# VanshJP/ShippingEnv

Measured on AMD Instinct MI355X. Metric: env-steps/sec at N=2^20 parallel envs per GPU (config 3: full step, 5 default ports; K steps in the steady state after a 1000-step pre-roll; config3_literal: the survey's 1000 steps from reset), higher is better.
Workload: dtype f64+int (fuel f64; reward computed in f64, stored f32 after one rounding; positions/cargo int)

## Files before the change

### shippingenv_amd/csrc/shipenv.hip

```cpp
#include <hip/hip_runtime.h>

#include <math.h>
#include <stdint.h>
#include <stdio.h>
#include <stdlib.h>
#include <string.h>

#include <algorithm>
#include <atomic>
#include <initializer_list>
#include <string>
#include <vector>

#include "../../include/shipenv.h"
#include "navfield.h"
#include "philox.h"
#include "step_lean.h"

#ifndef SHIPENV_TRACE
#define SHIPENV_TRACE 0
#endif

using namespace shipenv;

namespace {

constexpr int kBlock = 256;
constexpr int kStepBlock = 256;
constexpr int kEnvsPerThread = 4;
constexpr int kMaxBlocks = 2048;
constexpr int kStepBlocks = 32768;

constexpr uint32_t kUsedFuelGate = SE_USED_FUEL_GATE, kUsedLossType = SE_USED_LOSS_TYPE,
                   kUsedBeta = SE_USED_BETA, kUsedArrive = SE_USED_ARRIVE, kUsedMoved = SE_USED_MOVED;

constexpr double kFuelInit = 200.0;
constexpr double kMaxCargo = 50.0;

#include "world.h"
#include "env_core.h"
#include "step_io.h"
#include "step_group.h"
#include "step_agent.h"
#include "step_kernel.h"
#include "step_seq.h"
#include "views.h"
#include "rollout.h"
#include "episode.h"
#include "plan.h"
}

struct se_env {
    int device = 0;
    int64_t n = 0, env_base = 0;
    WorldDims dims{};
    uint64_t seed = 0;
    uint32_t flags = 0;
    uint64_t step_t = 0, epoch = 0;
    std::vector<uint8_t> water;
    std::vector<int32_t> port_x, port_y;
    uint32_t* d_world = nullptr;
    int64_t seg = 0;
    int64_t iters = 1;
    size_t world_cap = 0;
    uint64_t world_version = 0;
    int32_t cmax = 0, fmax = 0;
    int32_t stock_cargo_max = 0;
    se_state st{};
    bool bound = false;
    double* d_slab = nullptr;
    int32_t* d_offsets = nullptr;
    int grid = 0;
    int64_t nseg = 0;
    int64_t nslab = 0;
    uint8_t* d_mask_tmpl = nullptr;
    size_t mask_tmpl_cap = 0;
    uint64_t mask_tmpl_version = 0;
    int mask_ntmpl = 0;
    bool mask_tiled = false;
    int32_t done_pad = 1;
    bool nt_loads = false;
    bool seq_fuse = true;
    int32_t seq_max_steps = 1024;
    bool seq_gate_pool = true;
    bool seq_ring = true;
};

struct se_host {
    WorldDims dims{};
    std::vector<uint8_t> water;
    std::vector<uint32_t> img;
};

namespace {

#include "host.h"


int step_block_cap() {
    const char* v = getenv("SHIPENV_STEP_BLOCKS");
    const int c = v ? atoi(v) : 0;
    return c > 0 ? c : kStepBlocks;
}

int32_t done_pad_records(const se_env* env) {
    const char* v = getenv("SHIPENV_DONE_PAD");
    if (v) return atoi(v) == 0 ? 1 : 8;
    return env->n > (int64_t)1 << 23 ? 8 : 1;
}

bool step_nt_loads(const se_env* env) {
    const char* v = getenv("SHIPENV_NT_LOADS");
    if (v) return atoi(v) != 0;
    if (env->flags & SE_FLAG_AUTO_RESET) return env->n > (int64_t)1 << 21;
    return env->n <= (int64_t)1 << 23;
}

constexpr int32_t kSeqMaxSteps = 1024;
int32_t seq_max_steps() {
    const char* v = getenv("SHIPENV_SEQ_MAX_STEPS");
    const int c = v ? atoi(v) : 0;
    return c > 0 ? c : kSeqMaxSteps;
}
bool seq_fuse() {
    const char* v = getenv("SHIPENV_SEQ_FUSE");
    return !v || atoi(v) != 0;
}

bool seq_gate_pool() {
    const char* v = getenv("SHIPENV_SEQ_GATE_POOL");
    return !v || atoi(v) != 0;
}

bool seq_ring() {
    const char* v = getenv("SHIPENV_SEQ_RING");
    return !v || atoi(v) != 0;
}

bool mask_tiled() {
    const char* v = getenv("SHIPENV_MASK_TILED");
    return v && atoi(v) != 0;
}

int build_world_image(int H, int W, const std::vector<uint8_t>& water, int32_t P, const int32_t* px,
                      const int32_t* py, const int32_t* pf, const int32_t* pc, WorldDims& dims,
                      std::vector<uint32_t>& img) {
    if (P < 0 || P > SE_MAX_PORTS) return fail(SE_EINVAL, "P must be in [0, 254]");
    for (int i = 0; i < P; ++i) {
        if (px[i] < 0 || px[i] >= H || py[i] < 0 || py[i] >= W)
            return fail(SE_EINVAL, "Coordinates not within map");
        if (pf[i] < 0 || pc[i] < 0) return fail(SE_EINVAL, "port stocks must be >= 0");
    }
    const int cw = (H * W + 15) / 16 * 4;
    WorldDims d{H, W, P, cw};
    img.assign((size_t)d.padded(), 0u);
    uint8_t* cell = reinterpret_cast<uint8_t*>(img.data());
    for (int c = 0; c < H * W; ++c) cell[c] = water[c] ? 0 : (uint8_t)kCellGround;
    for (int i = P - 1; i >= 0; --i)
        cell[(size_t)px[i] * W + py[i]] = (uint8_t)(i + 1);
    for (int i = 0; i < P; ++i) {
        img[d.pos() + i] = (uint32_t)px[i] | ((uint32_t)py[i] << 16);
        img[d.stk() + 2 * i] = (uint32_t)pf[i];
        img[d.stk() + 2 * i + 1] = (uint32_t)pc[i];
    }
    for (int c = 0; c < 50; ++c) {
        const double q = (double)c / kMaxCargo;
        memcpy(&img[d.frac() + 2 * c], &q, sizeof q);
        img[d.gate() + c] = (uint32_t)floor(ldexp(q, 32));
    }
    img[d.gate() + 50] = 0xffffffffu;
    const int mdx[4] = {0, -1, 0, 1}, mdy[4] = {-1, 0, 1, 0};
    for (int k = 0; k < 4; ++k)
        img[d.moves() + k] = ((uint32_t)mdx[k] & 0xffffu) | (((uint32_t)mdy[k] & 0xffffu) << 16);
    double rtab[10];
    for (int k = 0; k < 8; ++k) {
        double r = 0.0;
        if (k & 4) r += -10.0;
        if (k & 2) {
            r += -5.0;
        } else {
            r += -0.0001;
            r += -1.0;
        }
        r += (k & 1) ? 2.0 : -2.0;
        rtab[k] = r;
    }
    rtab[8] = 0.05;
    rtab[9] = 0.0;
    memcpy(&img[d.rtab()], rtab, sizeof rtab);
    dims = d;
    return SE_OK;
}

int upload_world(se_env* env, int32_t P, const int32_t* px, const int32_t* py, const int32_t* pf,
                 const int32_t* pc) {
    WorldDims d{};
    std::vector<uint32_t> img;
    int rc = build_world_image(env->dims.H, env->dims.W, env->water, P, px, py, pf, pc, d, img);
    if (rc) return rc;
    std::vector<uint8_t> ring(ring_table_bytes(d.H, d.W));
    ring_table_build(d.H, d.W, reinterpret_cast<const uint8_t*>(img.data()), ring.data());
    rc = device_reserve(env->d_world, env->world_cap, (size_t)d.padded() * 4 + ring.size());
    if (rc) return rc;
    HIP_TRY(hipMemcpy(env->d_world, img.data(), (size_t)d.padded() * 4, hipMemcpyHostToDevice));
    HIP_TRY(hipMemcpy(env->d_world + d.padded(), ring.data(), ring.size(), hipMemcpyHostToDevice));
    env->dims = d;
    env->port_x.assign(px, px + P);
    env->port_y.assign(py, py + P);
    env->cmax = env->fmax = env->stock_cargo_max = 0;
    for (int i = 0; i < P; ++i) {
        env->cmax = std::max(env->cmax, std::min(pc[i], 49));
        env->fmax = std::max(env->fmax, std::min(pf[i], 199));
        env->stock_cargo_max = std::max(env->stock_cargo_max, pc[i]);
    }
    env->world_version += 1;
    env->mask_ntmpl = 1 + P;
    for (int p = 0; p < P; ++p)
        for (int q = 0; q < P; ++q) env->mask_ntmpl += (px[p] == px[q] && py[p] == py[q]) ? 1 : 0;
    return SE_OK;
}

typedef void (*StepFn)(StepArgs);
struct StepRow {
    uint32_t key;
    StepFn fn;
};
constexpr uint32_t step_key(bool typed, bool replay, bool autoreset, bool nt = false, bool rec = false, bool seq = false) {
    return typed | replay << 1 | autoreset << 2 | nt << 3 | rec << 4 | seq << 5;
}
template <bool... kFlags>
constexpr StepRow step_row() {
    return {step_key(kFlags...), step_kernel<kFlags...>};
}
template <bool... kFlags>
constexpr StepRow tail_row() {
    return {step_key(kFlags...), step_tail_kernel<kFlags...>};
}
constexpr StepRow kStepKernels[] = {
    step_row<false, false, false>(), step_row<false, false, false, true>(),
    step_row<false, false, true>(), step_row<false, false, true, true>(),
    step_row<false, false, false, false, false, true>(),
    step_row<false, false, false, true, false, true>(),
    step_row<false, false, true, false, true>(), step_row<false, false, true, true, true>(),
    step_row<false, true, false>(), step_row<true, true, false>(),
    step_row<true, false, false>(), step_row<true, false, true>(),
};
constexpr StepRow kStepTailKernels[] = {
    tail_row<false, false, false>(), tail_row<false, false, true>(), tail_row<false, true, false>(),
    tail_row<true, true, false>(),   tail_row<true, false, false>(), tail_row<true, false, true>(),
};

template <size_t kRows>
StepFn find_kernel(const StepRow (&rows)[kRows], uint32_t key) {
    for (const StepRow& r : rows)
        if (r.key == key) return r.fn;
    return nullptr;
}

StepArgs step_args(const se_env* env, const int32_t* act) {
    StepArgs A{};
    A.world = env->d_world;
    A.dims = env->dims;
    A.n = env->n;
    A.env_base = env->env_base;
    A.seed = env->seed;
    A.t = (uint32_t)env->step_t;
    A.st = env->st;
    A.act = act;
    A.iters = env->iters;
    return A;
}

int launch_step(se_env* env, bool typed, bool replay, const int32_t* act, const int32_t* a,
                const int32_t* b, se_tape* tape, void* stream, const StepRecord* rec = nullptr,
                bool seq = false) {
    int rc = check_ready(env);
    if (rc) return rc;
    if (env->n > 0 && (!act || (typed && (!a || !b)) || (replay && !tape)))
        return fail(SE_EINVAL, "null action/tape pointer");
    if (!aligned16(act) || (typed && (!aligned16(a) || !aligned16(b))))
        return fail(SE_EINVAL, "action buffers must be 16-byte aligned");
    const bool autoreset = (env->flags & SE_FLAG_AUTO_RESET) && !replay;
    if (autoreset && env->dims.P < 2) return fail(SE_EINVAL, "auto-reset needs at least two ports");
    DeviceGuard g(env->device);
    StepArgs A = step_args(env, act);
    A.act_a = a;
    A.act_b = b;
    A.tape = tape;
    if (autoreset) {
        const size_t par = (size_t)(env->step_t & 1u);
        A.done_recs = env->st.done_recs + par * (size_t)env->nseg * (size_t)env->seg;
        A.done_count = env->st.done_count + par * (size_t)env->nseg;
    }
    A.seg = env->seg;
    A.done_pad = env->done_pad;
    A.slab = env->d_slab;
    if (rec) A.rec = *rec;
    const bool agent = !typed && !replay;
    const StepFn full = find_kernel(kStepKernels, step_key(typed, replay, autoreset, agent && env->nt_loads,
                                                           rec != nullptr, agent && !autoreset && seq));
    const StepFn tail = find_kernel(kStepTailKernels, step_key(typed, replay, autoreset));
    if (!full || !tail) return fail(SE_EINVAL, "no step kernel for this kind of step");
    const hipStream_t s = (hipStream_t)stream;
    if (env->n >= kEnvsPerThread) {
        full<<<env->grid, kStepBlock, lds_bytes(env), s>>>(A);
        HIP_TRY(hipGetLastError());
    }
    if (env->n & 3) {
        tail<<<1, 64, 0, s>>>(A);
        HIP_TRY(hipGetLastError());
    }
    if (!replay) env->step_t += 1;
    return SE_OK;
}

int launch_step_seq(se_env* env, const int32_t* act, int64_t ld, int32_t steps, void* stream) {
    if (!act) return fail(SE_EINVAL, "null action/tape pointer");
    if (!aligned16(act)) return fail(SE_EINVAL, "action buffers must be 16-byte aligned");
    DeviceGuard g(env->device);
    const StepArgs A = step_args(env, act);
    const hipStream_t s = (hipStream_t)stream;
    if (env->n >= kEnvsPerThread) {
        const size_t base = lds_bytes(env) + kStockByCodeBytes;
        const bool pool = env->seq_gate_pool && base + kGatePoolBytes <= kLdsDefault;
        const size_t without = base + (pool ? kGatePoolBytes : 0);
        const uint32_t ring = env->seq_ring && ring_table_fits(env->dims.H, env->dims.W, env->dims.P, without)
                                  ? ring_table_bytes(env->dims.H, env->dims.W) : 0u;
        const size_t lds = without + ring;
        const auto kernel = pool ? (env->nt_loads ? step_seq_kernel<true, true> : step_seq_kernel<false, true>)
                                 : (env->nt_loads ? step_seq_kernel<true, false> : step_seq_kernel<false, false>);
        kernel<<<env->grid, kStepBlock, lds, s>>>(A, steps, ld, ring);
        HIP_TRY(hipGetLastError());
    }
    if (env->n & 3) {
        step_tail_seq_kernel<<<1, 64, 0, s>>>(A, steps, ld);
        HIP_TRY(hipGetLastError());
    }
    env->step_t += (uint64_t)steps;
    return SE_OK;
}

int launch_reset(se_env* env, const uint8_t* mask, const int32_t* origin, const int32_t* dest, void* stream) {
    if (env->n == 0) return SE_OK;
    DeviceGuard g(env->device);
    const ResetArgs A{env->d_world, env->dims, env->n, env->env_base, env->seed,
                      (uint32_t)env->epoch, (uint32_t)env->step_t, env->st, mask, origin, dest};
    reset_kernel<<<grid_for(env->n), kBlock, 0, (hipStream_t)stream>>>(A);
    HIP_TRY(hipGetLastError());
    return SE_OK;
}

}

void shipenv_set_error(const std::string& msg) { g_err = msg; }

extern "C" {

#if SHIPENV_TRACE
extern "C" int se_trace_read(void* host, size_t bytes) {
    return hipMemcpyFromSymbol(host, HIP_SYMBOL(g_trace), bytes) == hipSuccess ? 0 : -1;
}
#endif

int se_abi_version(void) { return SHIPENV_ABI_VERSION; }

const char* se_last_error(void) { return g_err.c_str(); }

int se_create(se_env** out, int device, int64_t n, int64_t env_id_base, int32_t H, int32_t W,
              const uint8_t* water, int32_t P, const int32_t* port_x, const int32_t* port_y,
              const int32_t* port_fuel, const int32_t* port_cargo, uint64_t seed, uint32_t flags) {
    if (!out) return fail(SE_EINVAL, "null out");
    *out = nullptr;
    if (n < 0) return fail(SE_EINVAL, "n must be >= 0");
    if (env_id_base < 0 || (env_id_base & 3))
        return fail(SE_EINVAL, "env_id_base must be a multiple of 4 (envs 4k..4k+3 share draw blocks)");
    if (H < 1 || W < 1 || H > SE_MAX_SIDE || W > SE_MAX_SIDE)
        return fail(SE_EINVAL, "map sides must be in [1, 256]");
    if (!water) return fail(SE_EINVAL, "null water map");
    if (P > 0 && (!port_x || !port_y || !port_fuel || !port_cargo))
        return fail(SE_EINVAL, "null port arrays");
    int ndev = 0;
    HIP_TRY(hipGetDeviceCount(&ndev));
    if (device < 0 || device >= ndev) return fail(SE_EINVAL, "bad device ordinal");
    DeviceGuard g(device);
    se_env* env = new se_env();
    env->device = device;
    env->n = n;
    env->env_base = env_id_base;
    env->seed = seed;
    env->flags = flags;
    env->dims.H = H;
    env->dims.W = W;
    env->water.assign(water, water + (size_t)H * W);
    for (auto& v : env->water) v = v ? 1 : 0;
    int rc = upload_world(env, P, port_x, port_y, port_fuel, port_cargo);
    if (rc) {
        se_destroy(env);
        return rc;
    }
    {
        const int64_t groups = (n + kEnvsPerThread - 1) / kEnvsPerThread;
        const int64_t cap = step_block_cap();
        env->iters = groups > 0 ? (groups + cap * kStepBlock - 1) / (cap * kStepBlock) : 1;
        env->grid = (int)(groups > 0 ? (groups + env->iters * kStepBlock - 1) / (env->iters * kStepBlock) : 1);
        env->seg = 64 * kEnvsPerThread;
        env->nseg = (int64_t)env->grid * env->iters * (kStepBlock / 64);
        env->nslab = (int64_t)env->grid * (kStepBlock / 64);
        env->done_pad = done_pad_records(env);
        env->nt_loads = step_nt_loads(env);
        env->seq_fuse = seq_fuse();
        env->seq_max_steps = seq_max_steps();
        env->seq_gate_pool = seq_gate_pool();
        env->seq_ring = seq_ring();
        env->mask_tiled = mask_tiled();
    }
    hipError_t e = hipMalloc(&env->d_slab, (size_t)env->nslab * 4 * sizeof(double));
    if (e == hipSuccess) e = hipMemset(env->d_slab, 0, (size_t)env->nslab * 4 * sizeof(double));
    if (e != hipSuccess) {
        se_destroy(env);
        return fail(SE_EHIP, std::string("se_create allocation: ") + hipGetErrorString(e));
    }
    *out = env;
    return SE_OK;
}

int se_set_ports(se_env* env, int32_t P, const int32_t* port_x, const int32_t* port_y,
                 const int32_t* port_fuel, const int32_t* port_cargo) {
    if (!env) return fail(SE_EINVAL, "null env");
    if (P > 0 && (!port_x || !port_y || !port_fuel || !port_cargo))
        return fail(SE_EINVAL, "null port arrays");
    DeviceGuard g(env->device);
    HIP_TRY(hipDeviceSynchronize());
    return upload_world(env, P, port_x, port_y, port_fuel, port_cargo);
}

int se_bind(se_env* env, const se_state* st) {
    if (!env || !st) return fail(SE_EINVAL, "null argument");
    const void* req[] = {st->x, st->y, st->fuel, st->cargo, st->origin, st->dest,
                         st->reward, st->done, st->err};
    for (const void* p : req) {
        if (!p && env->n > 0) return fail(SE_EINVAL, "null state buffer");
        if (!aligned16(p)) return fail(SE_EINVAL, "state buffers must be 16-byte aligned");
    }
    if (env->flags & SE_FLAG_AUTO_RESET) {
        if ((env->n > 0 && (!st->ep_return || !st->ep_start)) || !st->done_recs || !st->done_count)
            return fail(SE_EINVAL, "auto-reset needs ep_return, ep_start, done_recs and done_count");
        if (!aligned16(st->ep_return) || !aligned16(st->ep_start) || !aligned16(st->done_recs))
            return fail(SE_EINVAL, "state buffers must be 16-byte aligned");
        DeviceGuard g(env->device);
        HIP_TRY(hipMemset(st->done_count, 0, 2 * (size_t)env->nseg * sizeof(int32_t)));
    }
    env->st = *st;
    env->bound = true;
    return SE_OK;
}

int se_reset(se_env* env, const uint8_t* mask, void* stream) {
    int rc = check_ready(env);
    if (rc) return rc;
    if (env->dims.P < 2) return fail(SE_EINVAL, "reset needs at least two ports");
    rc = launch_reset(env, mask, nullptr, nullptr, stream);
    if (rc) return rc;
    env->epoch += 1;
    return SE_OK;
}

int se_reset_to(se_env* env, const uint8_t* mask, const int32_t* origin, const int32_t* dest,
                void* stream) {
    int rc = check_ready(env);
    if (rc) return rc;
    if (env->n > 0 && (!origin || !dest)) return fail(SE_EINVAL, "null origin/dest");
    return launch_reset(env, mask, origin, dest, stream);
}

int se_step(se_env* env, const int32_t* actions, void* stream) {
    return launch_step(env, false, false, actions, nullptr, nullptr, nullptr, stream);
}

int se_step_seq_mark(se_env* env, const int32_t* actions, int64_t ld, int32_t steps, void* stream,
                     void* event, int32_t mark_after) {
    int rc = check_ready(env);
    if (rc) return rc;
    if (steps < 0) return fail(SE_EINVAL, "negative step count");
    if (steps > 1 && (ld < env->n || (ld & 3))) return fail(SE_EINVAL, "row stride must be >= n and a multiple of 4");
    if (event && (mark_after < 0 || mark_after > steps)) return fail(SE_EINVAL, "mark_after must be in [0, steps]");
    const bool fused = env->seq_fuse && env->n > 0 && !(env->flags & SE_FLAG_AUTO_RESET) &&
                       lds_bytes(env) + kStockByCodeBytes <= kLdsDefault;
    for (int32_t k = 0; k <= steps;) {
        if (event && k == mark_after) {
            DeviceGuard g(env->device);
            HIP_TRY(hipEventRecord((hipEvent_t)event, (hipStream_t)stream));
        }
        if (k == steps) break;
        if (fused) {
            const int32_t end = event && k < mark_after ? mark_after : steps;
            const int32_t run = std::min(end - k, env->seq_max_steps);
            rc = launch_step_seq(env, actions + (int64_t)k * ld, ld, run, stream);
            k += run;
        } else {
            rc = launch_step(env, false, false, actions + (int64_t)k * ld, nullptr, nullptr, nullptr, stream, nullptr, true);
            k += 1;
        }
        if (rc) return rc;
    }
    return SE_OK;
}

int se_step_seq(se_env* env, const int32_t* actions, int64_t ld, int32_t steps, void* stream) {
    return se_step_seq_mark(env, actions, ld, steps, stream, nullptr, 0);
}

int se_step_typed(se_env* env, const int32_t* type, const int32_t* a, const int32_t* b,
                  void* stream) {
    return launch_step(env, true, false, type, a, b, nullptr, stream);
}

int se_step_replay(se_env* env, const int32_t* type, const int32_t* a, const int32_t* b,
                   se_tape* tape, void* stream) {
    return launch_step(env, true, true, type, a, b, tape, stream);
}

int se_step_agent_replay(se_env* env, const int32_t* actions, se_tape* tape, void* stream) {
    return launch_step(env, false, true, actions, nullptr, nullptr, tape, stream);
}

int se_observe(se_env* env, float* obs, int64_t ld, void* stream) {
    int rc = check_ready(env);
    if (rc) return rc;
    if ((env->n > 0 && !obs) || ld < 6 + 4 * (int64_t)env->dims.P) return fail(SE_EINVAL, "bad obs buffer / ld");
    DeviceGuard g(env->device);
    ObsArgs A{env->d_world, env->dims, env->n, ld, env->st, obs};
    const int64_t W = 6 + 4 * (int64_t)env->dims.P;
    const int64_t total = env->n * W;
    if (total == 0) return SE_OK;
    if (ld == W && aligned16(obs) && W <= 1022) {
        const uint32_t magic = (uint32_t)((((uint64_t)1 << 32) + (uint64_t)W - 1) / (uint64_t)W);
        const size_t lds = (size_t)(kTileRows * 6 + 4 * env->dims.P) * sizeof(float);
        observe_tiled_kernel<<<grid_for(env->n), kBlock, lds, (hipStream_t)stream>>>(A, magic);
    } else {
        observe_kernel<<<grid_for(total), kBlock, lds_bytes(env), (hipStream_t)stream>>>(A);
    }
    HIP_TRY(hipGetLastError());
    return SE_OK;
}

int se_valid_mask(se_env* env, uint8_t* bits, void* stream) {
    int rc = check_ready(env);
    if (rc) return rc;
    if (env->n > 0 && !bits) return fail(SE_EINVAL, "null bits");
    DeviceGuard g(env->device);
    const int32_t stride = (4 + env->dims.P + 250 + 7) / 8;
    MaskArgs A{env->d_world, env->dims, env->n, stride, env->st, bits};
    const int64_t total = env->n * stride;
    if (total == 0) return SE_OK;
    const hipStream_t s = (hipStream_t)stream;
    const int tb = mask_tb(stride);
    if (aligned16(bits) && env->dims.P <= 64 && env->mask_ntmpl <= kMaskTmplMax && !env->mask_tiled) {
        const size_t need = (size_t)kMaskHdr + (size_t)env->mask_ntmpl * tb;
        if (need > env->mask_tmpl_cap) env->mask_tmpl_version = 0;
        rc = device_reserve(env->d_mask_tmpl, env->mask_tmpl_cap, need);
        if (rc) return rc;
        if (env->mask_tmpl_version != env->world_version) {
            mask_tmpl_kernel<<<1, kBlock, 0, s>>>(env->d_world, env->dims, stride, env->d_mask_tmpl);
            HIP_TRY(hipGetLastError());
            env->mask_tmpl_version = env->world_version;
        }
// ... 257 lines not shown
```

### shippingenv_amd/csrc/step_lean.h

```cpp
#pragma once
#include <hip/hip_runtime.h>
#include <stdint.h>

namespace shipenv {

__host__ __device__ __forceinline__ bool lean_do_move(int act, int P, bool nodest, bool inb) {
    const bool is_mv = (uint32_t)act + 4u < (P != 0 ? 8u : 0u);
    return is_mv & !nodest & inb;
}
__host__ __device__ __forceinline__ uint32_t lean_move_bound(int P) {
    return P != 0 ? 0xFFFFFFF7u : 0xFFFFFFFFu;
}
__host__ __device__ __forceinline__ bool lean_do_move_val(int val, uint32_t bound, bool nodest, bool inb) {
    const bool is_mv = (uint32_t)val > bound;
    return is_mv & !nodest & inb;
}
__host__ __device__ __forceinline__ bool lean_sel_ok(int act, int P, bool same) {
    const bool is_sel = (uint32_t)act - 4u < (uint32_t)P;
    return is_sel & !same;
}

constexpr uint32_t kRingBorder = 254;
constexpr uint32_t kRingGround = 255;
constexpr int kRingMaxPorts = 253;
constexpr size_t kRingLdsPerBlock = 160 * 1024 / 4;
constexpr uint32_t kRingBias = 0x00010001u;

__host__ __device__ __forceinline__ uint32_t ring_table_bytes(int H, int W) {
    return ((uint32_t)(H + 2) * (uint32_t)(W + 2) + 15u) & ~15u;
}
__host__ __device__ __forceinline__ bool ring_table_fits(int H, int W, int P, size_t lds_without) {
    return P <= kRingMaxPorts && lds_without + ring_table_bytes(H, W) <= kRingLdsPerBlock;
}
__host__ __forceinline__ void ring_table_build(int H, int W, const uint8_t* cell, uint8_t* out) {
    const uint32_t n = ring_table_bytes(H, W);
    for (uint32_t i = 0; i < n; ++i) out[i] = i < (uint32_t)(H + 2) * (uint32_t)(W + 2) ? (uint8_t)kRingBorder : 0;
    for (int x = 0; x < H; ++x)
        for (int y = 0; y < W; ++y) out[(size_t)(x + 1) * (size_t)(W + 2) + (size_t)(y + 1)] = cell[(size_t)x * W + y];
}
__host__ __device__ __forceinline__ uint32_t ring_bias(uint32_t p) { return p + kRingBias; }
__host__ __device__ __forceinline__ uint32_t ring_unbias(uint32_t bp) { return bp - kRingBias; }
__host__ __device__ __forceinline__ uint32_t ring_index(uint32_t bp, int W) {
    return (bp & 0xffffu) * (uint32_t)(W + 2) + (bp >> 16);
}
__host__ __device__ __forceinline__ bool ring_do_move(int val, uint32_t bound, uint32_t code) {
    return ((uint32_t)val > bound) & (code != kRingBorder);
}
__host__ __device__ __forceinline__ bool ring_moved(int val, uint32_t bound, uint32_t code) {
    return ((uint32_t)val > bound) & (code < kRingBorder);
}

__host__ __device__ __forceinline__ double lean_fuel(double fuel, double scale, bool moved) {
    return __builtin_fma(-scale, moved ? 1.0 : 0.0, fuel);
}

__host__ __device__ __forceinline__ double lean_fuel_scale(uint32_t w, double fifth) {
    return 1.0 + __builtin_fma((double)w, fifth, -0.1);
}

__host__ __device__ __forceinline__ uint32_t gate_window_log2(uint32_t m) {
    return m <= 8 ? 3u : m <= 16 ? 2u : 1u;
}

}
```

### shippingenv_amd/csrc/step_seq.h

```cpp
#pragma once

struct Carried {
    uint32_t pos[4];
    int org[4], dst[4];
    uint32_t code[4];
    bool near;
    uint32_t thr[4];
    const int2* take;
};
__device__ __forceinline__ uint32_t gate_thr_of(const LdsWorld& w, int cargo) {
    return w.gate_thr[min(max(cargo, 0), 50)];
}
template <bool kSched>
struct SeqInv {
    KeySched ks;
    uint32_t move_bound;
    uint32_t ring0;
    __device__ __forceinline__ U4 block(const Key& qk, uint32_t t, uint32_t slot) const {
        if constexpr (kSched) return draw_sched(ks, qk, t, slot);
        else return draw(qk, t, slot);
    }
};
struct NoLateDraw {
    __device__ __forceinline__ void operator()(U4&) const {}
};
template <bool kNt, bool kSched, typename Late = NoLateDraw>
__device__ __forceinline__ bool step_group_state(const LdsWorld& w, const SeqInv<kSched>& I, const Key& qk, uint32_t t, U4 fb,
                                                 const U4& gb, Group<false, false, kNt>& G, Carried& U, Late late = Late{}) {
    const int P = w.P;
    const uint32_t lim = (uint32_t)(w.H - 1) | ((uint32_t)(w.W - 1) << 16);
    const uint32_t wh = (uint32_t)w.W | (1u << 16);
    const uint32_t pm1 = P > 0 ? (uint32_t)(P - 1) : 0u;
    bool take_any = false;
#pragma unroll
    for (int j = 0; j < 4; ++j) take_any |= (G.a[j] >= 4 + P) & (U.code[j] != 0);
    const bool take_ran = __builtin_amdgcn_ballot_w64(take_any) != 0;
    if (take_ran) {
#pragma unroll
        for (int j = 0; j < 4; ++j) {
            const int act = G.a[j];
            const bool lt_tc = act < 54 + P;
            const int amount = act - (lt_tc ? 4 + P : 54 + P);
            const int2 st2 = U.take[U.code[j]];
            const int stock = lt_tc ? st2.y : st2.x;
            const bool ok_take = (act >= 4 + P) & (amount > 0) & (amount <= stock);
            G.c[j] = (ok_take & lt_tc) ? G.c[j] + amount : G.c[j];
            G.f[j] = (ok_take & !lt_tc) ? G.f[j] + (double)amount : G.f[j];
            U.thr[j] = gate_thr_of(w, G.c[j]);
        }
    }
    late(fb);
    uint32_t pos[4], cp[4], code_cp[4];
    int dst[4], cg[4];
    bool do_move[4], moved[4], inb[4], nodest[4];
#pragma unroll
    for (int j = 0; j < 4; ++j) {
        const uint32_t dxy = w.moves[G.a[j] & 3];
        const uint32_t p = U.pos[j];
        dst[j] = U.dst[j];
        const uint32_t np = pk_add_u16(p, dxy);
        inb[j] = pk_min_u16(np, lim) == np;
        nodest[j] = dst[j] == SE_NONE;
        cp[j] = (!nodest[j] & inb[j]) ? np : p;
        code_cp[j] = lds_cell(lds_address(w.cell), cp[j], wh);
    }
    asm("" : "+v"(code_cp[0]), "+v"(code_cp[1]), "+v"(code_cp[2]), "+v"(code_cp[3]));
#pragma unroll
    for (int j = 0; j < 4; ++j) {
        const int act = G.a[j];
        const int val = (int)((uint32_t)act - 4u);
        const uint32_t p = U.pos[j];
        cg[j] = G.c[j];
        const bool ground = code_cp[j] == kCellGround;
        const bool same = U.org[j] == val;
        do_move[j] = lean_do_move_val(val, I.move_bound, nodest[j], inb[j]);
        moved[j] = do_move[j] & !ground;
        const bool sel_ok = lean_sel_ok(act, P, same);
        pos[j] = moved[j] ? cp[j] : p;
        U.code[j] = moved[j] ? code_cp[j] : U.code[j];
        dst[j] = sel_ok ? val : dst[j];
    }
    uint32_t fire = 0, arrive = 0;
    bool arrive_any = false;
#pragma unroll
    for (int j = 0; j < 4; ++j) arrive_any |= do_move[j] & (U.code[j] != 0);
    if (__builtin_amdgcn_ballot_w64(arrive_any) != 0) {
#pragma unroll
        for (int j = 0; j < 4; ++j)
            arrive |= (uint32_t)(do_move[j] & (pos[j] == w.pos[min((uint32_t)dst[j], pm1)])) << j;
    }
    double f[4];
#pragma unroll
    for (int j = 0; j < 4; ++j) {
        f[j] = lean_fuel(G.f[j], lean_fuel_scale(fb.v[j], kFifthPerWord), moved[j]);
        const bool fires = do_move[j] & (cg[j] > 0) & (gb.v[j] <= U.thr[j]);
        fire |= (uint32_t)fires << j;
    }
    asm volatile("" : "+v"(fire), "+v"(arrive));
    int org[4];
#pragma unroll
    for (int j = 0; j < 4; ++j) {
        org[j] = U.org[j];
        U.pos[j] = pos[j];
        G.f[j] = f[j];
    }
    if (fire) {
        uint32_t lt[4], v1[4], v2[4], v3[4];
        const uint32_t rk[4] = {0u, fire & 1u, (uint32_t)__popc(fire & 3u), (uint32_t)__popc(fire & 7u)};
        U4 rr = I.block(qk, t, loss_slot(0));
#pragma unroll
        for (int j = 0; j < 4; ++j) {
            lt[j] = rr.v[0];
            v1[j] = rr.v[1];
            v2[j] = rr.v[2];
            v3[j] = rr.v[3];
        }
#pragma unroll
        for (uint32_t q = 1; q < 4; ++q) {
            if (__popc(fire) > q) {
                rr = I.block(qk, t, loss_slot(q));
#pragma unroll
                for (int j = (int)q; j < 4; ++j) {
                    const bool take = rk[j] >= q;
                    lt[j] = take ? rr.v[0] : lt[j];
                    v1[j] = take ? rr.v[1] : v1[j];
                    v2[j] = take ? rr.v[2] : v2[j];
                    v3[j] = take ? rr.v[3] : v3[j];
                }
            }
        }
#pragma unroll
        for (int j = 0; j < 4; ++j) {
            if (__builtin_amdgcn_ballot_w64((fire >> j) & 1u) == 0) continue;
            const uint32_t lo = min(v1[j], v2[j]), hi = max(v1[j], v2[j]);
            const uint32_t med = max(lo, min(hi, v3[j]));
            const int part = beta_part(med, cg[j]);
            const int some = lt[j] > kTypeHi ? cg[j] : part;
            const int loss = lt[j] < kTypeLo ? 0 : some;
            const bool fj = (fire >> j) & 1u;
            cg[j] = fj ? cg[j] - loss : cg[j];
            U.thr[j] = gate_thr_of(w, cg[j]);
        }
    }
    if (arrive) {
        const U4 ab = I.block(qk, t, kSlotArrive);
#pragma unroll
        for (int j = 0; j < 4; ++j) {
            const bool aj = (arrive >> j) & 1u;
            const int nd = pick_other(ab.v[j], P, dst[j]);
            cg[j] = aj ? 0 : cg[j];
            U.thr[j] = gate_thr_of(w, cg[j]);
            org[j] = aj ? dst[j] : org[j];
            dst[j] = aj ? nd : dst[j];
        }
    }
#pragma unroll
    for (int j = 0; j < 4; ++j) {
        U.org[j] = org[j];
        U.dst[j] = dst[j];
        G.c[j] = cg[j];
    }
    return take_ran;
}

template <bool kNt, bool kSched, typename Late = NoLateDraw>
__device__ __forceinline__ bool step_group_ring(const LdsWorld& w, const SeqInv<kSched>& I, const Key& qk, uint32_t t, U4 fb,
                                                const U4& gb, Group<false, false, kNt>& G, Carried& U, Late late = Late{}) {
    const int P = w.P;
    const uint32_t wh = (uint32_t)(w.W + 2) | (1u << 16);
    const uint32_t pm1 = P > 0 ? (uint32_t)(P - 1) : 0u;
    bool take_ran = false;
    if (U.near) {
        bool take_any = false;
#pragma unroll
        for (int j = 0; j < 4; ++j) take_any |= (G.a[j] >= 4 + P) & (U.code[j] != 0);
        take_ran = __builtin_amdgcn_ballot_w64(take_any) != 0;
        if (take_ran) {
#pragma unroll
            for (int j = 0; j < 4; ++j) {
                const int act = G.a[j];
                const bool lt_tc = act < 54 + P;
                const int amount = act - (lt_tc ? 4 + P : 54 + P);
                const int2 st2 = U.take[U.code[j]];
                const int stock = lt_tc ? st2.y : st2.x;
                const bool ok_take = (act >= 4 + P) & (amount > 0) & (amount <= stock);
                G.c[j] = (ok_take & lt_tc) ? G.c[j] + amount : G.c[j];
                G.f[j] = (ok_take & !lt_tc) ? G.f[j] + (double)amount : G.f[j];
                U.thr[j] = gate_thr_of(w, G.c[j]);
            }
        }
    }
    late(fb);
    uint32_t np[4], code_t[4];
#pragma unroll
    for (int j = 0; j < 4; ++j) {
        np[j] = pk_add_u16(U.pos[j], w.moves[G.a[j] & 3]);
        code_t[j] = lds_cell(I.ring0, np[j], wh);
    }
    asm("" : "+v"(code_t[0]), "+v"(code_t[1]), "+v"(code_t[2]), "+v"(code_t[3]));
    int dst[4], cg[4];
    bool do_move[4], moved[4], fires[4];
    double f[4];
#pragma unroll
    for (int j = 0; j < 4; ++j) {
        const int act = G.a[j];
        const int val = (int)((uint32_t)act - 4u);
        cg[j] = G.c[j];
        const bool same = U.org[j] == val;
        do_move[j] = ring_do_move(val, I.move_bound, code_t[j]);
        moved[j] = ring_moved(val, I.move_bound, code_t[j]);
        const bool sel_ok = lean_sel_ok(act, P, same);
        U.pos[j] = moved[j] ? np[j] : U.pos[j];
        U.code[j] = moved[j] ? code_t[j] : U.code[j];
        dst[j] = sel_ok ? val : U.dst[j];
        f[j] = lean_fuel(G.f[j], lean_fuel_scale(fb.v[j], kFifthPerWord), moved[j]);
        fires[j] = do_move[j] & (cg[j] > 0) & (gb.v[j] <= U.thr[j]);
    }
    const bool near = __builtin_amdgcn_ballot_w64((U.code[0] | U.code[1] | U.code[2] | U.code[3]) != 0) != 0;
    U.near = near;
    uint32_t arrive = 0;
    if (near) {
#pragma unroll
        for (int j = 0; j < 4; ++j)
            arrive |= (uint32_t)(do_move[j] & (U.pos[j] == ring_bias(w.pos[min((uint32_t)dst[j], pm1)]))) << j;
    }
    int org[4];
#pragma unroll
    for (int j = 0; j < 4; ++j) {
        org[j] = U.org[j];
        G.f[j] = f[j];
    }
    if (__builtin_amdgcn_ballot_w64(fires[0] | fires[1] | fires[2] | fires[3]) != 0) {
        uint32_t fire = 0;
#pragma unroll
        for (int j = 0; j < 4; ++j) fire |= (uint32_t)fires[j] << j;
        asm volatile("" : "+v"(fire));
        uint32_t lt[4], v1[4], v2[4], v3[4];
        const uint32_t rk[4] = {0u, fire & 1u, (uint32_t)__popc(fire & 3u), (uint32_t)__popc(fire & 7u)};
        U4 rr = I.block(qk, t, loss_slot(0));
#pragma unroll
        for (int j = 0; j < 4; ++j) {
            lt[j] = rr.v[0];
            v1[j] = rr.v[1];
            v2[j] = rr.v[2];
            v3[j] = rr.v[3];
        }
#pragma unroll
        for (uint32_t q = 1; q < 4; ++q) {
            if (__popc(fire) > q) {
                rr = I.block(qk, t, loss_slot(q));
#pragma unroll
                for (int j = (int)q; j < 4; ++j) {
                    const bool take = rk[j] >= q;
                    lt[j] = take ? rr.v[0] : lt[j];
                    v1[j] = take ? rr.v[1] : v1[j];
                    v2[j] = take ? rr.v[2] : v2[j];
                    v3[j] = take ? rr.v[3] : v3[j];
                }
            }
        }
#pragma unroll
        for (int j = 0; j < 4; ++j) {
            if (__builtin_amdgcn_ballot_w64((fire >> j) & 1u) == 0) continue;
            const uint32_t lo = min(v1[j], v2[j]), hi = max(v1[j], v2[j]);
            const uint32_t med = max(lo, min(hi, v3[j]));
            const int part = beta_part(med, cg[j]);
            const int some = lt[j] > kTypeHi ? cg[j] : part;
            const int loss = lt[j] < kTypeLo ? 0 : some;
            const bool fj = (fire >> j) & 1u;
            cg[j] = fj ? cg[j] - loss : cg[j];
            U.thr[j] = gate_thr_of(w, cg[j]);
        }
    }
    if (arrive) {
        const U4 ab = I.block(qk, t, kSlotArrive);
#pragma unroll
        for (int j = 0; j < 4; ++j) {
            const bool aj = (arrive >> j) & 1u;
            const int nd = pick_other(ab.v[j], P, dst[j]);
            cg[j] = aj ? 0 : cg[j];
            U.thr[j] = gate_thr_of(w, cg[j]);
            org[j] = aj ? dst[j] : org[j];
            dst[j] = aj ? nd : dst[j];
        }
    }
#pragma unroll
    for (int j = 0; j < 4; ++j) {
        U.org[j] = org[j];
        U.dst[j] = dst[j];
        G.c[j] = cg[j];
    }
    return take_ran;
}

constexpr size_t kStockByCodeBytes = 256 * sizeof(int2);
static_assert(kStepBlock == 256, "stock_by_code: one cell code per thread");
__device__ __forceinline__ void stock_by_code(const LdsWorld& w, int2* take) {
    const uint32_t k = threadIdx.x - 1u, P = (uint32_t)w.P;
    const int2 s = w.stock[min(k, P > 0 ? P - 1 : 0u)];
    take[threadIdx.x] = k < P ? s : make_int2(0, 0);
}

constexpr uint32_t kGatePoolLimit = 16;
constexpr uint32_t kGatePoolSeeds = 32;
constexpr uint32_t kGatePoolRow = 64 + kGatePoolSeeds;
constexpr uint32_t kGateDirectRun = 16;
constexpr uint32_t kGateEarlyCut = 2;
constexpr size_t kGatePoolBytes = (kStepBlock / 64) * kGatePoolRow * sizeof(uint4);
constexpr int kRingRows = 3;
static_assert(kGatePoolLimit <= kGatePoolSeeds && kGatePoolLimit <= 32, "GATE pool: a window of at least 2 steps");

template <bool kOpaque>
__device__ __forceinline__ uint32_t seq_lane() {
    uint32_t lane = threadIdx.x;
    if constexpr (kOpaque) asm volatile("" : "+v"(lane));
    return lane;
}

template <bool kNt, bool kPool>
__global__ __launch_bounds__(kStepBlock) __attribute__((amdgpu_waves_per_eu(4))) void step_seq_kernel(
    StepArgs A, int32_t steps, int64_t ld, uint32_t ring_bytes) {
    extern __shared__ uint32_t lds[];
    if (steps <= 0) return;
    const uint32_t ring16 = steps > 1 ? ring_bytes >> 4 : 0u;
    const bool has_ring = ring16 != 0;
    const int64_t full = A.n >> 2;
    const int64_t first = (int64_t)blockIdx.x * A.iters * kStepBlock;

    const Staged st = stage_issue(A.world);
    __builtin_amdgcn_sched_barrier(0);
    Group<false, false, kNt> G;
    {
        const int64_t last = full - 1 - first;
        const uint32_t lane = last < (int64_t)threadIdx.x ? (uint32_t)(last < 0 ? 0 : last) : threadIdx.x;
        G.template load<true>(A, At<true>{last < 0 ? full - 1 : first, 0, A.n}, lane);
    }
    const uint4* const ring_g = reinterpret_cast<const uint4*>(A.world + A.dims.padded());
    const uint32_t ring_last = max(ring16, 1u) - 1u;
    const uint4 ring_r0 = ring_g[min(threadIdx.x, ring_last)];
    const uint4 ring_r1 = ring_g[min(threadIdx.x + kStepBlock, ring_last)];
    const uint4 ring_r2 = ring_g[min(threadIdx.x + 2 * kStepBlock, ring_last)];
    __builtin_amdgcn_sched_barrier(0);
    const LdsWorld w = stage_finish(A.world, A.dims, lds, st);
    int2* const take = reinterpret_cast<int2*>(lds + A.dims.padded());
    uint4* const gate_pool = reinterpret_cast<uint4*>(take + 256);
    uint4* const ring_l = reinterpret_cast<uint4*>(reinterpret_cast<uint8_t*>(take + 256) + (kPool ? kGatePoolBytes : 0));
    if (steps > 1) {
        stock_by_code(w, take);
        if (has_ring) {
            if (threadIdx.x < ring16) ring_l[threadIdx.x] = ring_r0;
            if (threadIdx.x + kStepBlock < ring16) ring_l[threadIdx.x + kStepBlock] = ring_r1;
            if (threadIdx.x + 2 * kStepBlock < ring16) ring_l[threadIdx.x + 2 * kStepBlock] = ring_r2;
            for (uint32_t i = threadIdx.x + kStepBlock * kRingRows; i < ring16; i += kStepBlock) ring_l[i] = ring_g[i];
        }
        __syncthreads();
    }

    SeqInv<kPool> I;
    if (steps > 1) {
        I.move_bound = lean_move_bound(w.P);
        asm volatile("" : "+s"(I.move_bound));
        I.ring0 = lds_address(reinterpret_cast<const uint8_t*>(ring_l));
    }

    BlockStats bs;
    Finished F;
    for (int64_t i = 0; i < A.iters; ++i) {
        const int64_t g0 = first + i * kStepBlock, g = g0 + threadIdx.x;
        if (g >= full) break;
        if (i > 0) {
            uint32_t lane = threadIdx.x;
            asm volatile("" : "+v"(lane));
            G.template load<true>(A, At<true>{g0, 0, A.n}, lane);
        }
        const uint32_t tl = A.t + (uint32_t)(steps - 1);
        if (steps > 1) {
            Carried U;
#pragma unroll
            for (int j = 0; j < 4; ++j) {
                U.pos[j] = unpack_pos(G.x, G.y, j);
                U.org[j] = byte_of(G.org, j);
                U.dst[j] = byte_of(G.dst, j);
                U.code[j] = w.cell[cell_of(U.pos[j], (uint32_t)w.W | (1u << 16))];
                U.thr[j] = gate_thr_of(w, G.c[j]);
            }
            U.take = take;
            bool irregular = false;
            {
                const uint32_t lim = (uint32_t)(w.H - 1) | ((uint32_t)(w.W - 1) << 16);
#pragma unroll
                for (int j = 0; j < 4; ++j) irregular |= (U.dst[j] == SE_NONE) | (pk_min_u16(U.pos[j], lim) != U.pos[j]);
            }
            const bool ring = has_ring && __builtin_amdgcn_ballot_w64(irregular) == 0;
            U.near = __builtin_amdgcn_ballot_w64((U.code[0] | U.code[1] | U.code[2] | U.code[3]) != 0) != 0;
            if (ring) {
#pragma unroll
                for (int j = 0; j < 4; ++j) U.pos[j] = ring_bias(U.pos[j]);
            }
            const Key qk = env_key(A.seed, (A.env_base + g * 4) >> 2);
            PairInv inv = pair_invariants(qk);
            asm volatile("" : "+v"(inv.hi[0]), "+v"(inv.lo[0]), "+v"(inv.hi[1]), "+v"(inv.lo[1]));
            const int32_t* row = A.act;
            if (!ring) {
                SeqInv<false> Ig;
                Ig.move_bound = I.move_bound;
                const uint32_t lane = seq_lane<kPool>();
                for (uint32_t t = A.t; t != tl; ++t) {
                    row += ld;
                    int32_t nxt[4];
                    ld4_full<kNt>(row, g0, nxt, lane);
                    const U4x2 fg = draw2(qk, inv, t);
                    step_group_state(w, Ig, qk, t, fg.fuel, fg.gate, G, U);
#pragma unroll
                    for (int j = 0; j < 4; ++j) G.a[j] = nxt[j];
                }
            } else if constexpr (!kPool) {
                for (uint32_t t = A.t; t != tl; ++t) {
                    row += ld;
                    int32_t nxt[4];
                    ld4_full<kNt>(row, g0, nxt);
                    const U4x2 fg = draw2(qk, inv, t);
                    step_group_ring(w, I, qk, t, fg.fuel, fg.gate, G, U);
#pragma unroll
                    for (int j = 0; j < 4; ++j) G.a[j] = nxt[j];
                }
            } else {
                {
                    const Key sk = env_key(A.seed, 0);
                    I.ks = key_schedule(sk.k0, sk.k1);
                    pin_schedule(I.ks);
                }
                const uint32_t lane = seq_lane<true>(), L = lane & 63u;
                uint4* const pool = gate_pool + (lane >> 6) * kGatePoolRow;
                uint4* const seeds = pool + 64;
                const bool whole = __builtin_amdgcn_ballot_w64(true) == ~0ull;
                uint32_t cuts = 0;
                for (uint32_t t = A.t; t != tl;) {
                    bool pooled = true;
                    do {
                        const bool carry = (G.c[0] > 0) | (G.c[1] > 0) | (G.c[2] > 0) | (G.c[3] > 0);
                        const uint64_t M = __builtin_amdgcn_ballot_w64(carry);
                        const uint32_t m = (uint32_t)__popcll(M);
                        if (!whole || m > kGatePoolLimit || (cuts >= 2 && m != 0)) {
                            pooled = false;
                            break;
                        }
                        const uint32_t logw = gate_window_log2(m);
                        const uint32_t slot = __builtin_amdgcn_mbcnt_hi((uint32_t)(M >> 32), __builtin_amdgcn_mbcnt_lo((uint32_t)M, 0u));
                        const uint32_t wmask = (1u << logw) - 1u;
                        if (m != 0) {
                            if (carry) seeds[slot] = make_uint4(inv.c3, inv.hi[1], inv.lo[1], qk.e1);
                            __builtin_amdgcn_fence(__ATOMIC_RELEASE, "wavefront");
                            __builtin_amdgcn_wave_barrier();
                            __builtin_amdgcn_fence(__ATOMIC_ACQUIRE, "wavefront");
                            const uint4 sd = seeds[min(L >> logw, m - 1u)];
                            const U4 gw = draw_gate_pooled_sched(I.ks, GateSeed{sd.x, sd.y, sd.z, sd.w}, t + (L & wmask));
                            pool[L] = make_uint4(gw.v[0], gw.v[1], gw.v[2], gw.v[3]);
                            __builtin_amdgcn_fence(__ATOMIC_RELEASE, "wavefront");
                            __builtin_amdgcn_wave_barrier();
                            __builtin_amdgcn_fence(__ATOMIC_ACQUIRE, "wavefront");
                        }
                        const uint4* const mine = pool + ((slot << logw) & 63u);
                        const uint32_t win = m != 0 ? min(tl - t, wmask + 1u) : tl - t;
                        uint32_t s = 0;
                        bool took;
                        do {
                            row += ld;
                            int32_t nxt[4];
                            ld4_full<kNt>(row, g0, nxt, lane);
                            const uint4 g4 = mine[s & wmask];
                            const auto fuel = [&](U4& fb) {
                                fb = draw_fuel_sched(I.ks, qk, inv, t);
                                asm volatile("" : "+v"(fb.v[0]), "+v"(fb.v[1]), "+v"(fb.v[2]), "+v"(fb.v[3]));
                            };
                            took = step_group_ring(w, I, qk, t, U4{}, U4{{g4.x, g4.y, g4.z, g4.w}}, G, U, fuel);
#pragma unroll
                            for (int j = 0; j < 4; ++j) G.a[j] = nxt[j];
                            ++s;
                            ++t;
                        } while (!took && s != win);
                        cuts = took && m != 0 && s <= kGateEarlyCut ? cuts + 1u : 0u;
                    } while (t != tl);
                    if (pooled) break;
                    cuts = min(cuts, 1u);
                    for (uint32_t n = min(tl - t, kGateDirectRun); n != 0; --n, ++t) {
                        row += ld;
                        int32_t nxt[4];
                        ld4_full<kNt>(row, g0, nxt, lane);
                        const U4x2 fg = draw2(qk, inv, t);
                        step_group_ring(w, I, qk, t, fg.fuel, fg.gate, G, U);
#pragma unroll
                        for (int j = 0; j < 4; ++j) G.a[j] = nxt[j];
                    }
                }
            }
            if (ring) {
#pragma unroll
                for (int j = 0; j < 4; ++j) U.pos[j] = ring_unbias(U.pos[j]);
            }
            pack_pos(U.pos, G.x, G.y);
            G.org = G.dst = 0;
#pragma unroll
            for (int j = 0; j < 4; ++j) {
                G.org |= (uint32_t)(U.org[j] & 0xff) << (8 * j);
                G.dst |= (uint32_t)(U.dst[j] & 0xff) << (8 * j);
            }
        }
        StepOut O;
        const uint32_t ln = seq_lane<true>();
        const At<true> at{g0, (g0 + ln) * 4, A.n};
        step_group_agent<false, true, kNt, false, false, true>(A, w, G, at, bs, F, early_draws<false>(A, at.base, tl), tl, &O);
        const se_state& S = late_args().st;
        __builtin_amdgcn_sched_barrier(0);
        st4u8_full(S.x, g0, G.x, ln);
        st4u8_full(S.y, g0, G.y, ln);
        st4_full(S.fuel, g0, G.f, ln);
        st4u8_full(S.done, g0, O.dn, ln);
        st4u8_full(reinterpret_cast<uint8_t*>(S.err), g0, O.ee, ln);
        __builtin_amdgcn_sched_barrier(0);
        st4u8_full(S.origin, g0, G.org, ln);
        st4u8_full(S.dest, g0, G.dst, ln);
        st4_full(S.cargo, g0, G.c, ln);
        st4_full(S.reward, g0, O.rw, ln);
    }
}

__global__ __launch_bounds__(64) void step_tail_seq_kernel(StepArgs A, int32_t steps, int64_t ld) {
    if (threadIdx.x != 0) return;
    const LdsWorld w = world_view(A.dims, A.world);
    const int32_t* act = A.act;
    const uint32_t t0 = A.t;
    for (int32_t k = 0; k < steps; ++k) {
        A.act = act + (int64_t)k * ld;
        A.t = t0 + (uint32_t)k;
        step_tail_envs<false, false, false>(A, w);
    }
}
```

Before: 733.4 billion.

## Screen pooled gate draws per step to skip fire evaluation on cold steps

When the gate pool draws its window of random words, each carrier's cargo thresholds are also written to LDS, and ballots build a per-step bitmask of steps where any lane's gate word could fire. In the pooled loop, the per-step fire computation (do_move, LDS read of the gate word, ballot) runs only when that step's screen bit is set; otherwise it is skipped. The gate threshold table construction moves into a shared helper. This adds extra LDS traffic and ballots during pool generation, and relies on the screen fold being correct for each window size. An environment variable can disable it.

```diff
diff --git a/shippingenv_amd/csrc/shipenv.hip b/shippingenv_amd/csrc/shipenv.hip
--- a/shippingenv_amd/csrc/shipenv.hip
+++ b/shippingenv_amd/csrc/shipenv.hip
@@ -84,6 +84,7 @@
     int32_t seq_max_steps = 1024;
     bool seq_gate_pool = true;
     bool seq_ring = true;
+    bool seq_screen = true;
 };
 
 struct se_host {
@@ -134,6 +135,11 @@
 
 bool seq_ring() {
     const char* v = getenv("SHIPENV_SEQ_RING");
+    return !v || atoi(v) != 0;
+}
+
+bool seq_screen() {
+    const char* v = getenv("SHIPENV_SEQ_SCREEN");
     return !v || atoi(v) != 0;
 }
 
@@ -166,9 +172,8 @@
     for (int c = 0; c < 50; ++c) {
         const double q = (double)c / kMaxCargo;
         memcpy(&img[d.frac() + 2 * c], &q, sizeof q);
-        img[d.gate() + c] = (uint32_t)floor(ldexp(q, 32));
-    }
-    img[d.gate() + 50] = 0xffffffffu;
+    }
+    for (int c = 0; c <= 50; ++c) img[d.gate() + c] = gate_thr_entry(c, kMaxCargo);
     const int mdx[4] = {0, -1, 0, 1}, mdy[4] = {-1, 0, 1, 0};
     for (int k = 0; k < 4; ++k)
         img[d.moves() + k] = ((uint32_t)mdx[k] & 0xffffu) | (((uint32_t)mdy[k] & 0xffffu) << 16);
@@ -329,7 +334,7 @@
         const size_t lds = without + ring;
         const auto kernel = pool ? (env->nt_loads ? step_seq_kernel<true, true> : step_seq_kernel<false, true>)
                                  : (env->nt_loads ? step_seq_kernel<true, false> : step_seq_kernel<false, false>);
-        kernel<<<env->grid, kStepBlock, lds, s>>>(A, steps, ld, ring);
+        kernel<<<env->grid, kStepBlock, lds, s>>>(A, steps, ld, ring, env->seq_screen ? 0u : ~0u);
         HIP_TRY(hipGetLastError());
     }
     if (env->n & 3) {
@@ -412,6 +417,7 @@
         env->seq_max_steps = seq_max_steps();
         env->seq_gate_pool = seq_gate_pool();
         env->seq_ring = seq_ring();
+        env->seq_screen = seq_screen();
         env->mask_tiled = mask_tiled();
     }
     hipError_t e = hipMalloc(&env->d_slab, (size_t)env->nslab * 4 * sizeof(double));
diff --git a/shippingenv_amd/csrc/step_lean.h b/shippingenv_amd/csrc/step_lean.h
--- a/shippingenv_amd/csrc/step_lean.h
+++ b/shippingenv_amd/csrc/step_lean.h
@@ -1,5 +1,6 @@
 #pragma once
 #include <hip/hip_runtime.h>
+#include <math.h>
 #include <stdint.h>
 
 namespace shipenv {
@@ -62,4 +63,20 @@
     return m <= 8 ? 3u : m <= 16 ? 2u : 1u;
 }
 
+__host__ __forceinline__ uint32_t gate_thr_entry(int c, double max_cargo) {
+    return c < (int)max_cargo ? (uint32_t)floor(ldexp((double)c / max_cargo, 32)) : 0xffffffffu;
 }
+
+__host__ __device__ __forceinline__ bool screen_hot(const uint32_t word[4], const uint32_t thr[4]) {
+    return (word[0] <= thr[0]) | (word[1] <= thr[1]) | (word[2] <= thr[2]) | (word[3] <= thr[3]);
+}
+__host__ __device__ __forceinline__ uint32_t screen_fold(uint64_t ballot, uint32_t logw) {
+    uint32_t b = (uint32_t)ballot | (uint32_t)(ballot >> 32);
+    b |= b >> 16;
+    b |= b >> 8;
+    b |= logw < 3u ? b >> 4 : 0u;
+    b |= logw < 2u ? b >> 2 : 0u;
+    return b;
+}
+
+}
diff --git a/shippingenv_amd/csrc/step_seq.h b/shippingenv_amd/csrc/step_seq.h
--- a/shippingenv_amd/csrc/step_seq.h
+++ b/shippingenv_amd/csrc/step_seq.h
@@ -163,9 +163,27 @@
     return take_ran;
 }
 
-template <bool kNt, bool kSched, typename Late = NoLateDraw>
+struct GateDrawn {
+    static constexpr bool kScreened = false;
+    const U4& gb;
+    __device__ __forceinline__ bool hot() const { return true; }
+    __device__ __forceinline__ U4 words() const { return gb; }
+};
+__device__ __forceinline__ uint32_t here(uint32_t v) {
+    asm volatile("" : "+v"(v));
+    return v;
+}
+template <typename Read>
+struct GateScreened {
+    static constexpr bool kScreened = true;
+    bool is_hot;
+    Read read;
+    __device__ __forceinline__ bool hot() const { return is_hot; }
+    __device__ __forceinline__ U4 words() const { return read(); }
+};
+template <bool kNt, bool kSched, typename Gate, typename Late = NoLateDraw>
 __device__ __forceinline__ bool step_group_ring(const LdsWorld& w, const SeqInv<kSched>& I, const Key& qk, uint32_t t, U4 fb,
-                                                const U4& gb, Group<false, false, kNt>& G, Carried& U, Late late = Late{}) {
+                                                const Gate& gate, Group<false, false, kNt>& G, Carried& U, Late late = Late{}) {
     const int P = w.P;
     const uint32_t wh = (uint32_t)(w.W + 2) | (1u << 16);
     const uint32_t pm1 = P > 0 ? (uint32_t)(P - 1) : 0u;
@@ -207,22 +225,24 @@
         const int val = (int)((uint32_t)act - 4u);
         cg[j] = G.c[j];
         const bool same = U.org[j] == val;
-        do_move[j] = ring_do_move(val, I.move_bound, code_t[j]);
+        if constexpr (!Gate::kScreened) do_move[j] = ring_do_move(val, I.move_bound, code_t[j]);
         moved[j] = ring_moved(val, I.move_bound, code_t[j]);
         const bool sel_ok = lean_sel_ok(act, P, same);
         U.pos[j] = moved[j] ? np[j] : U.pos[j];
         U.code[j] = moved[j] ? code_t[j] : U.code[j];
         dst[j] = sel_ok ? val : U.dst[j];
         f[j] = lean_fuel(G.f[j], lean_fuel_scale(fb.v[j], kFifthPerWord), moved[j]);
-        fires[j] = do_move[j] & (cg[j] > 0) & (gb.v[j] <= U.thr[j]);
+        if constexpr (!Gate::kScreened) fires[j] = do_move[j] & (cg[j] > 0) & (gate.words().v[j] <= U.thr[j]);
     }
     const bool near = __builtin_amdgcn_ballot_w64((U.code[0] | U.code[1] | U.code[2] | U.code[3]) != 0) != 0;
     U.near = near;
     uint32_t arrive = 0;
     if (near) {
 #pragma unroll
-        for (int j = 0; j < 4; ++j)
+        for (int j = 0; j < 4; ++j) {
+            if constexpr (Gate::kScreened) do_move[j] = ring_do_move((int)((uint32_t)G.a[j] - 4u), I.move_bound, here(code_t[j]));
             arrive |= (uint32_t)(do_move[j] & (U.pos[j] == ring_bias(w.pos[min((uint32_t)dst[j], pm1)]))) << j;
+        }
     }
     int org[4];
 #pragma unroll
@@ -230,7 +250,19 @@
         org[j] = U.org[j];
         G.f[j] = f[j];
     }
-    if (__builtin_amdgcn_ballot_w64(fires[0] | fires[1] | fires[2] | fires[3]) != 0) {
+    bool any_fire = false;
+    if constexpr (Gate::kScreened) {
+        if (gate.hot()) {
+            const U4 gb = gate.words();
+#pragma unroll
+            for (int j = 0; j < 4; ++j)
+                fires[j] = ring_do_move((int)((uint32_t)G.a[j] - 4u), I.move_bound, here(code_t[j])) & (cg[j] > 0) & (gb.v[j] <= U.thr[j]);
+            any_fire = __builtin_amdgcn_ballot_w64(fires[0] | fires[1] | fires[2] | fires[3]) != 0;
+        }
+    } else {
+        any_fire = __builtin_amdgcn_ballot_w64(fires[0] | fires[1] | fires[2] | fires[3]) != 0;
+    }
+    if (any_fire) {
         uint32_t fire = 0;
 #pragma unroll
         for (int j = 0; j < 4; ++j) fire |= (uint32_t)fires[j] << j;
@@ -309,6 +341,7 @@
 constexpr size_t kGatePoolBytes = (kStepBlock / 64) * kGatePoolRow * sizeof(uint4);
 constexpr int kRingRows = 3;
 static_assert(kGatePoolLimit <= kGatePoolSeeds && kGatePoolLimit <= 32, "GATE pool: a window of at least 2 steps");
+static_assert(2 * kGatePoolLimit <= kGatePoolSeeds, "GATE pool: the carriers' threshold rows follow their seed rows");
 
 template <bool kOpaque>
 __device__ __forceinline__ uint32_t seq_lane() {
@@ -319,7 +352,7 @@
 
 template <bool kNt, bool kPool>
 __global__ __launch_bounds__(kStepBlock) __attribute__((amdgpu_waves_per_eu(4))) void step_seq_kernel(
-    StepArgs A, int32_t steps, int64_t ld, uint32_t ring_bytes) {
+    StepArgs A, int32_t steps, int64_t ld, uint32_t ring_bytes, uint32_t screen_all) {
     extern __shared__ uint32_t lds[];
     if (steps <= 0) return;
     const uint32_t ring16 = steps > 1 ? ring_bytes >> 4 : 0u;
@@ -420,7 +453,7 @@
                     int32_t nxt[4];
                     ld4_full<kNt>(row, g0, nxt);
                     const U4x2 fg = draw2(qk, inv, t);
-                    step_group_ring(w, I, qk, t, fg.fuel, fg.gate, G, U);
+                    step_group_ring(w, I, qk, t, fg.fuel, GateDrawn{fg.gate}, G, U);
 #pragma unroll
                     for (int j = 0; j < 4; ++j) G.a[j] = nxt[j];
                 }
@@ -448,14 +481,23 @@
                         const uint32_t logw = gate_window_log2(m);
                         const uint32_t slot = __builtin_amdgcn_mbcnt_hi((uint32_t)(M >> 32), __builtin_amdgcn_mbcnt_lo((uint32_t)M, 0u));
                         const uint32_t wmask = (1u << logw) - 1u;
+                        uint32_t screen = screen_all;
                         if (m != 0) {
-                            if (carry) seeds[slot] = make_uint4(inv.c3, inv.hi[1], inv.lo[1], qk.e1);
+                            if (carry) {
+                                seeds[slot] = make_uint4(inv.c3, inv.hi[1], inv.lo[1], qk.e1);
+                                seeds[kGatePoolLimit + slot] = make_uint4(U.thr[0], U.thr[1], U.thr[2], U.thr[3]);
+                            }
                             __builtin_amdgcn_fence(__ATOMIC_RELEASE, "wavefront");
                             __builtin_amdgcn_wave_barrier();
                             __builtin_amdgcn_fence(__ATOMIC_ACQUIRE, "wavefront");
-                            const uint4 sd = seeds[min(L >> logw, m - 1u)];
+                            const uint32_t of = min(L >> logw, m - 1u);
+                            const uint4 sd = seeds[of];
+                            const uint4 th = seeds[kGatePoolLimit + of];
                             const U4 gw = draw_gate_pooled_sched(I.ks, GateSeed{sd.x, sd.y, sd.z, sd.w}, t + (L & wmask));
                             pool[L] = make_uint4(gw.v[0], gw.v[1], gw.v[2], gw.v[3]);
+                            const uint64_t hot = __builtin_amdgcn_ballot_w64(gw.v[0] <= th.x) | __builtin_amdgcn_ballot_w64(gw.v[1] <= th.y) |
+                                                 __builtin_amdgcn_ballot_w64(gw.v[2] <= th.z) | __builtin_amdgcn_ballot_w64(gw.v[3] <= th.w);
+                            screen |= screen_fold(hot, logw);
                             __builtin_amdgcn_fence(__ATOMIC_RELEASE, "wavefront");
                             __builtin_amdgcn_wave_barrier();
                             __builtin_amdgcn_fence(__ATOMIC_ACQUIRE, "wavefront");
@@ -468,12 +510,15 @@
                             row += ld;
                             int32_t nxt[4];
                             ld4_full<kNt>(row, g0, nxt, lane);
-                            const uint4 g4 = mine[s & wmask];
+                            const auto words = [&]() {
+                                const uint4 g4 = mine[s & wmask];
+                                return U4{{g4.x, g4.y, g4.z, g4.w}};
+                            };
                             const auto fuel = [&](U4& fb) {
                                 fb = draw_fuel_sched(I.ks, qk, inv, t);
                                 asm volatile("" : "+v"(fb.v[0]), "+v"(fb.v[1]), "+v"(fb.v[2]), "+v"(fb.v[3]));
                             };
-                            took = step_group_ring(w, I, qk, t, U4{}, U4{{g4.x, g4.y, g4.z, g4.w}}, G, U, fuel);
+                            took = step_group_ring(w, I, qk, t, U4{}, GateScreened<decltype(words)>{((screen >> (s & 31u)) & 1u) != 0, words}, G, U, fuel);
 #pragma unroll
                             for (int j = 0; j < 4; ++j) G.a[j] = nxt[j];
                             ++s;
@@ -488,7 +533,7 @@
                         int32_t nxt[4];
                         ld4_full<kNt>(row, g0, nxt, lane);
                         const U4x2 fg = draw2(qk, inv, t);
-                        step_group_ring(w, I, qk, t, fg.fuel, fg.gate, G, U);
+                        step_group_ring(w, I, qk, t, fg.fuel, GateDrawn{fg.gate}, G, U);
 #pragma unroll
                         for (int j = 0; j < 4; ++j) G.a[j] = nxt[j];
                     }
```

Result: faster. 783.1 billion (median of 6 runs) (+6.8%).
